# ShawnHuang497/MedPLIB

Hardware: AMD Instinct MI355X
Metric: train samples/sec (img+64tok) (higher is better)
Workload: dtype bf16

## Files before the change

### include/medplib_hip.h

```cpp
#ifndef MEDPLIB_HIP_H
#define MEDPLIB_HIP_H
#include <stddef.h>
#include <stdint.h>

#ifdef __cplusplus
extern "C" {
#endif

typedef struct ihipStream_t* hipStream_t;

#define MP_OK 0
#define MP_ERR_SHAPE (-1)
#define MP_ERR_DTYPE (-2)
#define MP_ERR_WORKSPACE (-3)
#define MP_ERR_LAUNCH (-4)
#define MP_ERR_ARG (-5)
#define MP_BF16 0
#define MP_F32 1
#define MP_ACT_NONE 0
#define MP_ACT_RELU 1
#define MP_ACT_GELU 2
#define MP_ACT_QUICK_GELU 3
#define MP_ACT_SILU 4
#define MP_ACT_SWIGLU_PAIR 5

int mp_version(void);
const char* mp_arch(void);
const char* mp_last_error_string(void);
int mp_profile_marker(int tag, hipStream_t stream);


int mp_gemm_bf16_nt(const void* A, int64_t lda, const void* W, int64_t ldw, void* C, int64_t ldc, const float* bias,
                    const void* residual, int64_t ldr, int M, int N, int K, int act, int out_dtype, float alpha,
                    const int* m_dev, hipStream_t stream);
int mp_gemm_qkv_rope_bf16(const void* A, int64_t lda, const void* Wi, int64_t ldw, void* C, int64_t ldc, const float* cos_t,
                          const float* sin_t, int M, int N, int K, int seq, int pos_offset, int head_dim, hipStream_t stream);
int mp_gemm_qkv_rope_bounded_bf16(const void* A, int64_t lda, const void* Wi, int64_t ldw, void* C, int64_t ldc, const float* cos_t,
                                  const float* sin_t, int M, int N, int K, int seq, int pos_offset, int head_dim, int table_rows,
                                  hipStream_t stream);
int mp_gemm_swiglu_keep_bf16(const void* A, int64_t lda, const void* W, int64_t ldw, void* act_out, int64_t ld_act, void* gu_out,
                             int64_t ld_gu, int M, int N, int K, hipStream_t stream);
int mp_gemm_last_kernel(void);
int mp_gemm_tile_policy(int mode);
int64_t mp_gemm_tail_wait(int64_t cycles);
int mp_gemm_bf16_nt_batched(const void* A, int64_t lda, int64_t strideA, const void* W, int64_t ldw, int64_t strideW,
                            void* C, int64_t ldc, int64_t strideC, const float* bias, int64_t strideBias, int batch,
                            int M, int N, int K, int act, int out_dtype, const int* m_dev, hipStream_t stream);

int mp_gemm_bf16_nt_batched_res(const void* A, int64_t lda, int64_t strideA, const void* W, int64_t ldw, int64_t strideW, void* C,
                                int64_t ldc, int64_t strideC, const void* residual, int64_t ldr, int64_t strideR, int batch, int M, int N,
                                int K, const int* m_dev, hipStream_t stream);

int mp_gemm_bf16_nt_batched_rows(const void* A, int64_t lda, int64_t strideA, const int* a_rows, const void* W, int64_t ldw,
                                 int64_t strideW, void* C, int64_t ldc, int64_t strideC, const int* c_rows, const float* c_scale,
                                 const void* residual, int64_t ldr, int rows_stride, int batch, int M, int N, int K, int act,
                                 const int* m_dev, hipStream_t stream);

int mp_gemv_bf16(const void* x, int64_t ldx, const void* W, int64_t ldw, int64_t strideW, void* y, int64_t ldy, const float* bias,
                 const void* residual, int64_t ldr, const int* w_index, const float* row_scale, const int* row_keep, int M, int N, int K,
                 int act, int out_dtype, float alpha, hipStream_t stream);
int mp_gemv_top2_gate_up_bf16(const void* x, int64_t ldx, const void* W, int64_t ldw, int64_t strideW, void* act, int64_t ldact,
                              const int* expert, const int* slot, int tokens, int N, int K, hipStream_t stream);
int mp_gemv_top2_down_bf16(const void* act, int64_t ldact, const void* W, int64_t ldw, int64_t strideW, void* y, int64_t ldy,
                           const void* residual, int64_t ldr, const int* expert, const int* slot, const float* weight, int tokens, int N,
                           int K, hipStream_t stream);
int mp_gemv_rmsnorm_bf16(const void* x, int64_t ldx, const float* norm_w, float eps, const void* W, int64_t ldw, void* y, int64_t ldy,
                         int M, int N, int K, int act, int out_dtype, hipStream_t stream);
int mp_gemv_rmsnorm_rope_append_bf16(const void* x, int64_t ldx, const float* norm_w, float eps, const void* W_qkv, int64_t ldw, void* qkv,
                                     int64_t ldy, const float* cos_t, const float* sin_t, void* cache_k, void* cache_v, const int* pos_dev,
                                     int M, int heads, int head_dim, int K, int64_t cache_batch_stride, int64_t cache_seq_stride,
                                     hipStream_t stream);
#define MP_POS_ERR_TABLE 1
#define MP_POS_ERR_CACHE 2
#define MP_POS_ERR_BEAM 4
int mp_gemv_rmsnorm_rope_append_bounded_bf16(const void* x, int64_t ldx, const float* norm_w, float eps, const void* W_qkv, int64_t ldw,
                                             void* qkv, int64_t ldy, const float* cos_t, const float* sin_t, void* cache_k, void* cache_v,
                                             const int* pos_dev, int M, int heads, int head_dim, int K, int64_t cache_batch_stride,
// ... 293 lines not shown
```

### medplib_amd/csrc/gemm320_bf16.hip

```cpp
#include "gemm_common.h"
#include <stdlib.h>
#include <algorithm>

namespace {

constexpr int BM3 = 320, BN3 = 256, BK3 = 64, NT3 = 512;
constexpr int A_BYTES = BM3 * 128, B_BYTES = BN3 * 128, STAGE3 = A_BYTES + B_BYTES;

__device__ __forceinline__ int lds_off3(int r, int c) { return r * 128 + ((c ^ (r & 7)) << 4); }

#define MP3_BAR()                          \
  do {                                     \
    asm volatile("" ::: "memory");         \
    __builtin_amdgcn_sched_barrier(0);     \
    __builtin_amdgcn_s_barrier();          \
    __builtin_amdgcn_sched_barrier(0);     \
    asm volatile("" ::: "memory");         \
  } while (0)
#define MP3_LGKM0() asm volatile("s_waitcnt lgkmcnt(0)" ::: "memory")

constexpr int EPI_PLAIN = 0, EPI_ROPE = 1, EPI_SWIGLU = 2, EPI_COMBINE = 3, EPI_RELU = 4, EPI_GELU = 5;
template <int EPI>
__device__ __forceinline__ void gemm320_epilogue(const GemmArgs& g, f32x4 (&acc)[5][8], int batch, int M, int N, int m0, int n0, int wr, int wc,
                                                 int fr, int fq, unsigned items = 0xfffffu) {
  bf16_t* Cb = reinterpret_cast<bf16_t*>(g.C) + batch * g.sC;
  const int cw = n0 + wc * 128;
  const int c8 = pair_col8(fq);
  if constexpr (EPI == EPI_SWIGLU) {
    float rsc[5] = {1.f, 1.f, 1.f, 1.f, 1.f};
    if (g.a_scale) {
#pragma unroll
      for (int i = 0; i < 5; ++i) {
        const int row = m0 + wr * 80 + i * 16 + fr;
        if (row < M) rsc[i] = g.a_scale[g.a_rows ? g.a_rows[batch * g.rows_stride + row] : row];
      }
    }
#pragma unroll
    for (int i = 0; i < 5; ++i) {
      const int row = m0 + wr * 80 + i * 16 + fr;
#pragma unroll
      for (int jb = 0; jb < 2; ++jb) {
        if (!((items >> (i * 4 + jb * 2)) & 1u)) continue;
        bf16x4 o[2];
#pragma unroll
        for (int jj = 0; jj < 2; ++jj)
#pragma unroll
          for (int r = 0; r < 4; ++r) {
            acc[i][jb * 4 + jj][r] *= rsc[i];
            acc[i][jb * 4 + jj + 2][r] *= rsc[i];
            const float gf = (float)(bf16_t)acc[i][jb * 4 + jj][r];
            const float uf = (float)(bf16_t)acc[i][jb * 4 + jj + 2][r];
            o[jj][r] = (bf16_t)(gf * mp_sigmoid_fast(gf) * uf);
          }
        const bf16x8 p = pair_swap16(o[0], o[1]);
        if (row < M) *reinterpret_cast<bf16x8*>(Cb + (int64_t)row * g.ldc + (cw >> 1) + jb * 32 + c8) = p;
        if (g.keep_gu) {
          const bf16x8 pg = pair_swap16(round4(acc[i][jb * 4]), round4(acc[i][jb * 4 + 1])), pu = pair_swap16(round4(acc[i][jb * 4 + 2]), round4(acc[i][jb * 4 + 3]));
          if (row < M) {
            *reinterpret_cast<bf16x8*>(g.keep_gu + (int64_t)row * g.ld_gu + cw + jb * 64 + c8) = pg;
            *reinterpret_cast<bf16x8*>(g.keep_gu + (int64_t)row * g.ld_gu + cw + jb * 64 + 32 + c8) = pu;
          }
        }
      }
      __builtin_amdgcn_sched_barrier(0);
    }
    return;
  }
  if constexpr (EPI == EPI_COMBINE) {
    bf16_t* Cs = reinterpret_cast<bf16_t*>(g.C);
    int orow[5];
    float sc[5];
#pragma unroll
    for (int i = 0; i < 5; ++i) {
      const int row = m0 + wr * 80 + i * 16 + fr;
      orow[i] = row < M ? g.c_rows[batch * g.rows_stride + row] : -1;
    }
#pragma unroll
    for (int i = 0; i < 5; ++i) sc[i] = (orow[i] >= 0 && g.c_scale) ? g.c_scale[orow[i]] : 1.f;
#pragma unroll
    for (int h = 0; h < 2; ++h) {
      bf16x8 rv[5][2];
#pragma unroll
      for (int i = 0; i < 5; ++i)
#pragma unroll
        for (int jp = 0; jp < 2; ++jp) {
          const int col = cw + (h * 2 + jp) * 32 + c8;
          rv[i][jp] = bf16x8{};
          if (g.residual && orow[i] >= 0 && ((items >> (i * 4 + h * 2 + jp)) & 1u))
            rv[i][jp] = *reinterpret_cast<const bf16x8*>(g.residual + (int64_t)orow[i] * g.ldr + col);
        }
      __builtin_amdgcn_sched_barrier(0);
#pragma unroll
      for (int i = 0; i < 5; ++i)
#pragma unroll
        for (int jp = 0; jp < 2; ++jp) {
          const int col = cw + (h * 2 + jp) * 32 + c8;
          const bf16x8 p = pair_swap16(round4(acc[i][(h * 2 + jp) * 2]), round4(acc[i][(h * 2 + jp) * 2 + 1]));
          bf16x8 o;
#pragma unroll
          for (int e = 0; e < 8; ++e) {
            float v = (float)p[e] * sc[i];
            if (g.residual) v += (float)rv[i][jp][e];
            o[e] = (bf16_t)v;
          }
          if (orow[i] >= 0 && ((items >> (i * 4 + h * 2 + jp)) & 1u)) *reinterpret_cast<bf16x8*>(Cs + (int64_t)orow[i] * g.ldc + col) = o;
        }
      __builtin_amdgcn_sched_barrier(0);
    }
    return;
  }
  if constexpr (EPI == EPI_ROPE) {
    const bool is_v = n0 >= (N / 3) * 2;
    const int head0 = (cw >> 7) << 7;
    f32x4 cs[2][2][2], sn[2][2][2];
    float rsc[2] = {1.f, 1.f};
    auto fetch = [&](int i, int buf) {
      const int row = m0 + wr * 80 + i * 16 + fr;
      const int pos = (row < M ? row : 0) % g.rope_seq + g.rope_pos0;
      if (g.a_scale) rsc[buf] = g.a_scale[row < M ? row : 0];
#pragma unroll
      for (int jb = 0; jb < 2; ++jb)
#pragma unroll
        for (int jj = 0; jj < 2; ++jj) {
          const int dim = jb * 32 + jj * 16 + fq * 4;
          cs[buf][jb][jj] = *reinterpret_cast<const f32x4*>(g.rope_cos + (int64_t)pos * 64 + dim);
          sn[buf][jb][jj] = *reinterpret_cast<const f32x4*>(g.rope_sin + (int64_t)pos * 64 + dim);
        }
    };
    fetch(0, 0);
#pragma unroll
    for (int i = 0; i < 5; ++i) {
      if (i + 1 < 5) fetch(i + 1, (i + 1) & 1);
      __builtin_amdgcn_sched_barrier(0);
      const int row = m0 + wr * 80 + i * 16 + fr;
#pragma unroll
      for (int jb = 0; jb < 2; ++jb) {
        bf16x4 olo[2], ohi[2];
#pragma unroll
        for (int jj = 0; jj < 2; ++jj) {
          const bf16x4 qa = round4(acc[i][jb * 4 + jj] * rsc[i & 1]), qb = round4(acc[i][jb * 4 + jj + 2] * rsc[i & 1]);
#pragma unroll
          for (int r = 0; r < 4; ++r) {
            const float a = (float)qa[r], b = (float)qb[r];
            const bf16_t rlo = (bf16_t)(a * cs[i & 1][jb][jj][r] - b * sn[i & 1][jb][jj][r]);
            const bf16_t rhi = (bf16_t)(b * cs[i & 1][jb][jj][r] + a * sn[i & 1][jb][jj][r]);
            olo[jj][r] = is_v ? qa[r] : rlo;
            ohi[jj][r] = is_v ? qb[r] : rhi;
          }
        }
        const bf16x8 plo = pair_swap16(olo[0], olo[1]), phi = pair_swap16(ohi[0], ohi[1]);
        const int col_lo = (is_v ? cw + jb * 64 : head0 + jb * 32) + c8;
        const int col_hi = (is_v ? cw + jb * 64 + 32 : head0 + 64 + jb * 32) + c8;
        if (row < M) {
          *reinterpret_cast<bf16x8*>(Cb + (int64_t)row * g.ldc + col_lo) = plo;
          *reinterpret_cast<bf16x8*>(Cb + (int64_t)row * g.ldc + col_hi) = phi;
        }
      }
      __builtin_amdgcn_sched_barrier(0);
    }
    return;
  }
  const float* bias0 = g.bias ? g.bias + batch * g.sBias : nullptr;
  if (g.alpha != 1.f || bias0) {
#pragma unroll
    for (int j = 0; j < 8; ++j) {
      f32x4 bv = {0.f, 0.f, 0.f, 0.f};
      if (bias0) {
#pragma unroll
        for (int r = 0; r < 4; ++r) { const int col = cw + j * 16 + fq * 4 + r; bv[r] = col < N ? bias0[col] : 0.f; }
      }
#pragma unroll
      for (int i = 0; i < 5; ++i) acc[i][j] = acc[i][j] * g.alpha + bv;
    }
  }
#define MP3_ACT_SWEEP(EXPR)                                                          \
  _Pragma("unroll") for (int i = 0; i < 5; ++i) _Pragma("unroll") for (int j = 0; j < 8; ++j) {                    \
    _Pragma("unroll") for (int r = 0; r < 4; ++r) { const float v = acc[i][j][r]; acc[i][j][r] = (EXPR); }         \
    __builtin_amdgcn_sched_barrier(0);                                                                             \
  }
  if constexpr (EPI == EPI_RELU) { MP3_ACT_SWEEP(fmaxf(v, 0.f)) }
  else if constexpr (EPI == EPI_GELU) { MP3_ACT_SWEEP(gelu_erf_fast(v)) }
  else if (g.act == ACT_QUICK_GELU) { MP3_ACT_SWEEP(v * mp_sigmoid_fast(v, 1.702f)) }
#undef MP3_ACT_SWEEP
  const bf16_t* R = g.residual ? g.residual + batch * g.sR : nullptr;
#pragma unroll
  for (int h = 0; h < 2; ++h) {
    bf16x8 rv[5][2];
    if (R) {
#pragma unroll
      for (int i = 0; i < 5; ++i) {
        const int row = m0 + wr * 80 + i * 16 + fr;
#pragma unroll
        for (int jp = 0; jp < 2; ++jp) {
          const int col = cw + (h * 2 + jp) * 32 + c8;
          rv[i][jp] = bf16x8{};
          if (row < M && col < N && ((items >> (i * 4 + h * 2 + jp)) & 1u)) rv[i][jp] = *reinterpret_cast<const bf16x8*>(R + (int64_t)row * g.ldr + col);
        }
      }
      __builtin_amdgcn_sched_barrier(0);
    }
#pragma unroll
    for (int i = 0; i < 5; ++i) {
      const int row = m0 + wr * 80 + i * 16 + fr;
#pragma unroll
      for (int jp = 0; jp < 2; ++jp) {
        const int col = cw + (h * 2 + jp) * 32 + c8;
        bf16x8 p = pair_swap16(round4(acc[i][(h * 2 + jp) * 2]), round4(acc[i][(h * 2 + jp) * 2 + 1]));
        if (R) {
#pragma unroll
          for (int e = 0; e < 8; ++e) p[e] = (bf16_t)((float)p[e] + (float)rv[i][jp][e]);
        }
        if (row < M && col < N && ((items >> (i * 4 + h * 2 + jp)) & 1u)) *reinterpret_cast<bf16x8*>(Cb + (int64_t)row * g.ldc + col) = p;
      }
    }
    __builtin_amdgcn_sched_barrier(0);
  }
}

constexpr int MAX_FLAT_BATCH3 = 8;
template <int EPI>
__global__ __launch_bounds__(NT3, 1) void gemm320_bf16_nt_kernel(GemmArgs g) {
  extern __shared__ __attribute__((aligned(16))) char smem[];
  const int N = g.N;
  const int tiles_n = N / BN3;
  int T = 0;
  int pre[MAX_FLAT_BATCH3];
#pragma unroll
  for (int b = 0; b < MAX_FLAT_BATCH3; ++b) {
    pre[b] = T;
    if (b < g.nbatch) {
      const int Mb = g.m_dev ? min(g.M, g.m_dev[b * g.m_dev_stride]) : g.M;
      T += ((Mb + BM3 - 1) / BM3) * tiles_n;
    }
  }
  const int C = g.n_cu;
  const int full = (T / C) * C, rem = T - full;
  const int nt_all = g.K / BK3;
  int S = 1;
  if (g.ws && rem > 0 && rem * 2 <= C) S = max(1, min(min(min(C / rem, g.max_split), nt_all / 4), EPI == EPI_SWIGLU ? 10 : 20));
  const int bid = blockIdx.x;
  if (bid >= full + rem * S) return;
  int flat, split = 0;
  if (bid < full) {
    flat = (bid & 7) * (full >> 3) + (bid >> 3);
  } else {
    const int r = bid - full;
    if (S == 1 && (rem & 7) == 0) {
      flat = full + (r & 7) * (rem >> 3) + (r >> 3);
    } else {
      flat = full + r % rem;
      split = r / rem;
    }
  }
  const bool is_split = (bid >= full) && S > 1;
  int batch = 0, pbase = 0;
#pragma unroll
  for (int b = 1; b < MAX_FLAT_BATCH3; ++b) if (b < g.nbatch && flat >= pre[b]) { batch = b; pbase = pre[b]; }
  const int lid = flat - pbase;
  const int M = g.m_dev ? min(g.M, g.m_dev[batch * g.m_dev_stride]) : g.M;
  const int tiles_m = (M + BM3 - 1) / BM3;
  const int GROUP_M = g.group_m;
  const int per_group = GROUP_M * tiles_n;
  const int grp = lid / per_group;
  const int first_m = grp * GROUP_M;
  const int gsz = min(tiles_m - first_m, GROUP_M);
  const int tm = first_m + (lid % per_group) % gsz, tn = (lid % per_group) / gsz;
  const int m0 = tm * BM3, n0 = tn * BN3;
  int kt0 = 0, nt = nt_all;
  if (is_split) {
    const int base = nt_all / S, extra = nt_all % S;
    kt0 = split * base + min(split, extra);
    nt = base + (split < extra ? 1 : 0);
  }
  const int k_byte0 = kt0 * (BK3 * 2);

  const int tid = threadIdx.x;
  const int lane = tid & 63;
  const int wave = __builtin_amdgcn_readfirstlane(tid >> 6);
  const int wc = wave >> 2, wr = wave & 3;
  const int fr = lane & 15, fq = lane >> 4;

  const int sub_row = lane >> 3;
  const int src_c = (lane & 7) ^ sub_row;
  const __amdgpu_buffer_rsrc_t rs_a = __builtin_amdgcn_make_buffer_rsrc(const_cast<bf16_t*>(g.A + batch * g.sA), 0,
                                          g.a_rows ? 0x7ffffff0 : (int)(((int64_t)(M - 1) * g.lda + g.K) * 2), 0x00020000);
  const __amdgpu_buffer_rsrc_t rs_w = __builtin_amdgcn_make_buffer_rsrc(const_cast<bf16_t*>(g.W + batch * g.sW), 0, (int)(((int64_t)(N - 1) * g.ldw + g.K) * 2), 0x00020000);
  const int w_lane = (int)((sub_row * g.ldw + src_c * 8) * 2);
  const int w_row_bytes = (int)(g.ldw * 2);
  int a_off[5];
#pragma unroll
  for (int i = 0; i < 5; ++i) {
    int row = m0 + (wave + 8 * i) * 8 + sub_row;
    if (g.a_rows) row = g.a_rows[batch * g.rows_stride + min(row, M - 1)];
    a_off[i] = (int)(((int64_t)row * g.lda + src_c * 8) * 2);
  }
  int b_piece[4];
#pragma unroll
  for (int k = 0; k < 4; ++k) {
    const int e = 2 * wave + (k & 1);
    b_piece[k] = (e & 7) + (e >> 3) * 16 + (k >> 1) * 8;
  }
  auto dma_a = [&](int i, int t) {
    __builtin_amdgcn_raw_ptr_buffer_load_lds(rs_a, (__attribute__((address_space(3))) void*)(smem + (t & 1) * STAGE3 + (wave + 8 * i) * 1024), 16,
                                             a_off[i], k_byte0 + t * (BK3 * 2), 0, 0);
  };
  auto dma_b = [&](int k, int t) {
    __builtin_amdgcn_raw_ptr_buffer_load_lds(rs_w, (__attribute__((address_space(3))) void*)(smem + (t & 1) * STAGE3 + A_BYTES + b_piece[k] * 1024), 16,
                                             w_lane, (n0 + b_piece[k] * 8) * w_row_bytes + k_byte0 + t * (BK3 * 2), 0, 0);
  };

  f32x4 acc[5][8];
#pragma unroll
  for (int i = 0; i < 5; ++i)
#pragma unroll
    for (int j = 0; j < 8; ++j) acc[i][j] = f32x4{0.f, 0.f, 0.f, 0.f};
  bf16x8 fa[5][2], fb[4][2];
  const int a_rd0 = (wr * 80 + fr) * 128 + ((fq ^ (fr & 7)) << 4), a_rd1 = (wr * 80 + fr) * 128 + (((4 + fq) ^ (fr & 7)) << 4);
  const int b_rd0 = A_BYTES + (wc * 128 + fr) * 128 + ((fq ^ (fr & 7)) << 4), b_rd1 = A_BYTES + (wc * 128 + fr) * 128 + (((4 + fq) ^ (fr & 7)) << 4);
  auto load_a = [&](const char* st) {
#pragma unroll
    for (int i = 0; i < 5; ++i) {
      fa[i][0] = *reinterpret_cast<const bf16x8*>(st + a_rd0 + i * 2048);
      fa[i][1] = *reinterpret_cast<const bf16x8*>(st + a_rd1 + i * 2048);
    }
  };
  auto load_b = [&](int hn, const char* st) {
#pragma unroll
    for (int j = 0; j < 4; ++j) {
      fb[j][0] = *reinterpret_cast<const bf16x8*>(st + b_rd0 + (hn * 64 + j * 16) * 128);
      fb[j][1] = *reinterpret_cast<const bf16x8*>(st + b_rd1 + (hn * 64 + j * 16) * 128);
    }
  };
#ifndef MP3_PRIO
#define MP3_PRIO 0
#endif
#define MP3_MFMA_40(HN)                                                                                     \
  do {                                                                                                      \
    if (MP3_PRIO == 0) __builtin_amdgcn_s_setprio(1);                                                       \
    _Pragma("unroll") for (int kk = 0; kk < 2; ++kk)                                                        \
      _Pragma("unroll") for (int i = 0; i < 5; ++i)                                                         \
        _Pragma("unroll") for (int j = 0; j < 4; ++j)                                                       \
          acc[i][(HN) * 4 + j] = __builtin_amdgcn_mfma_f32_16x16x32_bf16(fb[j][kk], fa[i][kk], acc[i][(HN) * 4 + j], 0, 0, 0); \
    if (MP3_PRIO == 0) __builtin_amdgcn_s_setprio(0);                                                       \
    MP3_BAR();                                                                                              \
  } while (0)

#pragma unroll
  for (int i = 0; i < 5; ++i) dma_a(i, 0);
#pragma unroll
  for (int k = 0; k < 4; ++k) dma_b(k, 0);
  if (nt > 1) {
#pragma unroll
    for (int i = 0; i < 5; ++i) dma_a(i, 1);
    dma_b(0, 1); dma_b(1, 1);
    asm volatile("s_waitcnt vmcnt(7)" ::: "memory");
  } else {
    asm volatile("s_waitcnt vmcnt(0)" ::: "memory");
  }
  MP3_BAR();
  if (wc == 1) MP3_BAR();
  if (MP3_PRIO == 2 && wc == 1) __builtin_amdgcn_s_setprio(1);

  for (int t = 0; t < nt; ++t) {
    const char* st = smem + (t & 1) * STAGE3;
    const bool n1 = (t + 1 < nt), n2 = (t + 2 < nt);
    load_b(0, st);
    load_a(st);
    __builtin_amdgcn_sched_barrier(0);
    if (n1) { dma_b(2, t + 1); dma_b(3, t + 1); }
    MP3_LGKM0();
    MP3_BAR();
    MP3_MFMA_40(0);
    load_b(1, st);
    __builtin_amdgcn_sched_barrier(0);
    if (n2) {
#pragma unroll
      for (int i = 0; i < 5; ++i) dma_a(i, t + 2);
      dma_b(0, t + 2); dma_b(1, t + 2);
      asm volatile("s_waitcnt vmcnt(7)" ::: "memory");
    } else {
      asm volatile("s_waitcnt vmcnt(0)" ::: "memory");
    }
    MP3_LGKM0();
    MP3_BAR();
    MP3_MFMA_40(1);
  }
  if (wc == 0) MP3_BAR();
  if (MP3_PRIO == 2) __builtin_amdgcn_s_setprio(0);
  unsigned items = 0xfffffu;
  if (is_split) {
    typedef __attribute__((ext_vector_type(4))) unsigned int u32x4;
    constexpr int SLAB = BM3 * BN3 * 4;
    const int tail = flat - full;
    float* tile_ws = g.ws + ((int64_t)tail * S) * (BM3 * BN3);
    const __amdgpu_buffer_rsrc_t rs = __builtin_amdgcn_make_buffer_rsrc(tile_ws, 0, S * SLAB, 0x00020000);
    const int my_off = split * SLAB + tid * 16;
#pragma unroll
    for (int i = 0; i < 5; ++i)
#pragma unroll
      for (int j = 0; j < 8; ++j)
        __builtin_amdgcn_raw_buffer_store_b128(__builtin_bit_cast(u32x4, acc[i][j]), rs, my_off + (i * 8 + j) * (NT3 * 16), 0, 16);
    asm volatile("s_waitcnt vmcnt(0)" ::: "memory");
    __syncthreads();
    int* arrive = g.tickets + tail;
    int* depart = g.tickets + 128 + tail;
    int* mode = g.tickets + 256 + tail;
    constexpr int MODE_COOP = 1, MODE_LAST = 2;
    int* s_flag = reinterpret_cast<int*>(smem);
    if (tid == 0) {
      __hip_atomic_fetch_add(arrive, 1, __ATOMIC_RELAXED, __HIP_MEMORY_SCOPE_AGENT);
      const long long t0 = __builtin_amdgcn_s_memtime();
      int m = 0, seen = 0;
      for (;;) {
        seen = __hip_atomic_load(arrive, __ATOMIC_RELAXED, __HIP_MEMORY_SCOPE_AGENT);
        if (seen >= S) break;
        m = __hip_atomic_load(mode, __ATOMIC_RELAXED, __HIP_MEMORY_SCOPE_AGENT);
        if (m) break;
        if (__builtin_amdgcn_s_memtime() - t0 > g.tail_wait) break;
        __builtin_amdgcn_s_sleep(8);
      }
      if (!m) {
        int expected = 0;
        const int want = seen >= S ? MODE_COOP : MODE_LAST;
        m = __hip_atomic_compare_exchange_strong(mode, &expected, want, __ATOMIC_RELAXED, __ATOMIC_RELAXED, __HIP_MEMORY_SCOPE_AGENT) ? want : expected;
      }
      int last = 0;
      if (m == MODE_LAST) last = __hip_atomic_fetch_add(depart, 1, __ATOMIC_RELAXED, __HIP_MEMORY_SCOPE_AGENT) == S - 1;
      s_flag[0] = m | (last << 8);
    }
    __syncthreads();
    const int decided = s_flag[0];
    __syncthreads();
    const bool coop = (decided & 0xff) == MODE_COOP;
    if (!coop && !(decided >> 8)) return;
    constexpr int N_ITEMS = (EPI == EPI_SWIGLU) ? 10 : 20;
    items = 0;
#pragma unroll
    for (int it = 0; it < N_ITEMS; ++it)
      if (!coop || it % S == split) items |= (EPI == EPI_SWIGLU) ? (3u << (2 * it)) : (1u << it);
#pragma unroll
    for (int i = 0; i < 5; ++i)
#pragma unroll
      for (int j = 0; j < 8; ++j) acc[i][j] = f32x4{0.f, 0.f, 0.f, 0.f};
    for (int sp = 0; sp < S; ++sp) {
      const int base = sp * SLAB + tid * 16;
#pragma unroll
      for (int it = 0; it < 20; ++it) {
        if (!((items >> it) & 1u)) continue;
        const int i = it >> 2, j0 = (it & 3) * 2;
        u32x4 t[2];
#pragma unroll
        for (int q = 0; q < 2; ++q) t[q] = __builtin_amdgcn_raw_buffer_load_b128(rs, base + (i * 8 + j0 + q) * (NT3 * 16), 0, 16);
#pragma unroll
        for (int q = 0; q < 2; ++q) acc[i][j0 + q] += __builtin_bit_cast(f32x4, t[q]);
      }
    }
    asm volatile("s_waitcnt vmcnt(0)" ::: "memory");
    __syncthreads();
    if (tid == 0) {
      const bool rearm = coop ? (__hip_atomic_fetch_add(depart, 1, __ATOMIC_RELAXED, __HIP_MEMORY_SCOPE_AGENT) == S - 1) : true;
      if (rearm) {
        __hip_atomic_store(depart, 0, __ATOMIC_RELAXED, __HIP_MEMORY_SCOPE_AGENT);
        __hip_atomic_store(mode, 0, __ATOMIC_RELAXED, __HIP_MEMORY_SCOPE_AGENT);
        __hip_atomic_store(arrive, 0, __ATOMIC_RELAXED, __HIP_MEMORY_SCOPE_AGENT);
      }
    }
  }
  int tid2 = threadIdx.x;
  asm volatile("" : "+v"(tid2));
  gemm320_epilogue<EPI>(g, acc, batch, M, N, m0, n0, (tid2 >> 6) & 3, tid2 >> 8, tid2 & 15, (tid2 >> 4) & 3, items);
}

}

bool mp_gemm320_eligible(const GemmArgs& g, int batch) {
  if (batch < 1 || batch > MAX_FLAT_BATCH3 || g.out_f32) return false;
  if (g.keep_gu && (batch != 1 || (g.ld_gu & 7) || (reinterpret_cast<uintptr_t>(g.keep_gu) & 15))) return false;
  if (!(g.act == ACT_NONE || g.act == ACT_QUICK_GELU || g.act == ACT_ROPE_QK || g.act == ACT_SWIGLU_PAIR || g.act == ACT_RELU || g.act == ACT_GELU)) return false;
  if ((g.act == ACT_RELU || g.act == ACT_GELU) && (g.c_rows || g.a_rows)) return false;
  if (g.act == ACT_ROPE_QK && (batch != 1 || g.m_dev || g.a_rows || g.c_rows)) return false;
  if (g.act == ACT_SWIGLU_PAIR && (g.c_rows || g.residual || g.bias || g.alpha != 1.f || ((g.N >> 1) & 7))) return false;
  if (g.c_rows && (g.act != ACT_NONE || g.bias || g.alpha != 1.f)) return false;
  if (g.a_scale && !(g.act == ACT_ROPE_QK || g.act == ACT_SWIGLU_PAIR)) return false;
  if (g.N % BN3 || g.K % BK3 || g.M < (mp_gemm_policy_whole_tiles() ? BM3 : 1024)) return false;
  if ((g.ldc & 7) || (reinterpret_cast<uintptr_t>(g.C) & 15) || (g.sC & 7)) return false;
  if (g.residual && ((g.ldr & 7) || (reinterpret_cast<uintptr_t>(g.residual) & 15) || (g.sR & 7))) return false;
  const int64_t a_rows_bound = g.a_rows ? (int64_t)batch * g.M * 4 : (int64_t)g.M + 320;
  if (a_rows_bound * g.lda * 2 >= (1ll << 31) || (int64_t)g.N * g.ldw * 2 >= (1ll << 31)) return false;
  return true;
}

int mp_gemm320_subwave_split(const GemmArgs& g, int batch) {
  static int on = -1;
  if (on < 0) { const char* e = getenv("MP_GEMM320_SUBWAVE"); on = (e && atoi(e) == 0) ? 0 : 1; }
  if (!on || batch != 1 || g.m_dev || g.act == ACT_ROPE_QK || g.M < 1024 || g.K < 8192) return 1;
  if (mp_gemm_policy_whole_tiles()) return 1;
  const int C = std::min(mp_device_cus(), 256);
  const int64_t tiles = (int64_t)mp_cdiv(g.M, BM3) * (g.N / BN3);
  if (tiles * 2 > C || tiles * 4 <= C) return 1;
  const int64_t S = std::min<int64_t>(C / tiles, g.K / BK3 / 4);
  if (S < 2 || S * tiles * 10 < (int64_t)C * 9) return 1;
  return (int)S;
}

int mp_launch_gemm320(const GemmArgs& g0, int batch, hipStream_t stream) {
  static bool attr = false;
  if (!attr) {
    (void)hipFuncSetAttribute((const void*)gemm320_bf16_nt_kernel<EPI_PLAIN>, hipFuncAttributeMaxDynamicSharedMemorySize, 2 * STAGE3);
    (void)hipFuncSetAttribute((const void*)gemm320_bf16_nt_kernel<EPI_ROPE>, hipFuncAttributeMaxDynamicSharedMemorySize, 2 * STAGE3);
    (void)hipFuncSetAttribute((const void*)gemm320_bf16_nt_kernel<EPI_SWIGLU>, hipFuncAttributeMaxDynamicSharedMemorySize, 2 * STAGE3);
    (void)hipFuncSetAttribute((const void*)gemm320_bf16_nt_kernel<EPI_COMBINE>, hipFuncAttributeMaxDynamicSharedMemorySize, 2 * STAGE3);
    (void)hipFuncSetAttribute((const void*)gemm320_bf16_nt_kernel<EPI_RELU>, hipFuncAttributeMaxDynamicSharedMemorySize, 2 * STAGE3);
    (void)hipFuncSetAttribute((const void*)gemm320_bf16_nt_kernel<EPI_GELU>, hipFuncAttributeMaxDynamicSharedMemorySize, 2 * STAGE3);
    attr = true;
  }
  GemmArgs g = g0;
  g.nbatch = batch;
  g.n_cu = std::min(mp_device_cus(), 256);
  static int max_split = -1;
  if (max_split < 0) { const char* e = getenv("MP_GEMM320_MAX_SPLIT"); max_split = (e && atoi(e) >= 1) ? atoi(e) : 10; }
  static int dense_split = -1;
  if (dense_split < 0) { const char* e = getenv("MP_GEMM320_DENSE_SPLIT"); dense_split = (e && atoi(e) == 0) ? 0 : 1; }
  const int64_t dense_tiles = (int64_t)mp_cdiv(g.M, BM3) * (g.N / BN3);
  g.max_split = (batch > 1 || g.m_dev) ? max_split : ((dense_split && (dense_tiles > g.n_cu || mp_gemm320_subwave_split(g, batch) > 1)) ? max_split : 1);
  if (g.act == ACT_ROPE_QK) g.max_split = 1;
  if (mp_gemm_stream_registered(stream) || mp_gemm_policy_whole_tiles()) g.max_split = 1;
  g.tail_wait = mp_gemm_tail_wait_value();
  int64_t ws_bytes = 0;
  mp_gemm_split_workspace(stream, &g.ws, &g.tickets, &ws_bytes);
  if (!g.ws || ws_bytes < (int64_t)g.n_cu * BM3 * BN3 * 4) { g.ws = nullptr; g.tickets = nullptr; g.max_split = 1; }
  const int64_t host_tiles = (int64_t)mp_cdiv(g.M, BM3) * (g.N / BN3) * batch;
  const int64_t host_rem = host_tiles % g.n_cu;
  const bool may_split = g.max_split > 1 && (g.m_dev || (host_rem > 0 && host_rem * 2 <= g.n_cu));
  const dim3 grid((unsigned)(host_tiles + (may_split ? g.n_cu : 0)));
#define MP3_GO(E) hipLaunchKernelGGL(gemm320_bf16_nt_kernel<E>, grid, dim3(NT3), 2 * STAGE3, stream, g)
  if (g.act == ACT_ROPE_QK) MP3_GO(EPI_ROPE);
  else if (g.act == ACT_SWIGLU_PAIR) MP3_GO(EPI_SWIGLU);
  else if (g.c_rows) MP3_GO(EPI_COMBINE);
  else if (g.act == ACT_RELU) MP3_GO(EPI_RELU);
  else if (g.act == ACT_GELU) MP3_GO(EPI_GELU);
  else MP3_GO(EPI_PLAIN);
#undef MP3_GO
  return mp_check_launch("mp_gemm_bf16_nt(320)");
}
```

### medplib_amd/csrc/gemm_common.h

```cpp
#pragma once
#include "common.h"

enum { ACT_NONE = 0, ACT_RELU = 1, ACT_GELU = 2, ACT_QUICK_GELU = 3, ACT_SILU = 4,
       ACT_SWIGLU_PAIR = 5,
       ACT_ROPE_QK = 6 };

struct GemmArgs {
  const bf16_t* A;  int64_t lda;
  const bf16_t* W;  int64_t ldw;
  void* C;          int64_t ldc;
  const float* bias;
  const bf16_t* residual;
  int64_t ldr;
  const int* m_dev;
  int M, N, K;
  int act;
  int out_f32;
  float alpha;
  int64_t sA, sW, sC, sR, sBias;
  int m_dev_stride;
  int group_m;
  float* ws; int* tickets;
  int n_cu;
  int nbatch;
  int max_split;
  long long tail_wait;
  const int* a_rows; const int* c_rows; const float* c_scale;
  int rows_stride;
  const float* rope_cos; const float* rope_sin;
  int rope_seq, rope_pos0;
  int ep8;
  bf16_t* keep_gu; int64_t ld_gu;
  const float* a_scale;
};

static __device__ __forceinline__ float gelu_erf_fast(float x) {
  const float xp = fmaxf(x, 0.f);
  const float a = fabsf(x);
  float q = fmaf(-0.0004733088717330247f, a, 0.007084553129971027f);
  q = fmaf(q, a, -0.05182736739516258f);
  q = fmaf(q, a, -0.4599924683570862f);
  q = fmaf(q, a, -1.1507878303527832f);
  q = fmaf(q, a, -1.000037670135498f);
  return fmaf(-a, __builtin_amdgcn_exp2f(q), xp);
}

static __device__ __forceinline__ float apply_act(float v, int act) {
  switch (act) {
    case ACT_RELU: return fmaxf(v, 0.f);
    case ACT_GELU: return gelu_erf_fast(v);
    case ACT_QUICK_GELU: return v * mp_sigmoid_fast(v, 1.702f);
    case ACT_SILU: return v * mp_sigmoid_fast(v);
    default: return v;
  }
}


void mp_launch_gemm128(const GemmArgs& g, int batch, bool may_split, hipStream_t stream);
int mp_launch_gemm256(const GemmArgs& g, int batch, hipStream_t stream);
// ... 21 lines not shown
```

### medplib_amd/ops.py

```python
import torch

from ._lib import lib

BF16, F32 = 0, 1
ACT_NONE, ACT_RELU, ACT_GELU, ACT_QUICK_GELU, ACT_SILU, ACT_SWIGLU_PAIR = 0, 1, 2, 3, 4, 5
SACT_NONE, SACT_RELU, SACT_GELU, SACT_SIGMOID = 0, 1, 2, 3


def _stream():
    return torch.cuda.current_stream().cuda_stream


def _p(t):
    return None if t is None else t.data_ptr()


def _chk(t, dtype, name):
    if not t.is_cuda:
        raise ValueError(f"{name}: expected a GPU tensor (medplib_amd has no CPU path)")
    if t.dtype != dtype:
        raise TypeError(f"{name}: expected {dtype}, got {t.dtype}")


def _dt(dtype):
# ... 161 lines not shown
    import functools

    @functools.wraps(fn)
    def wrapped(*args, **kwargs):
        with throughput_tiles():
            return fn(*args, **kwargs)
    return wrapped


class throughput_tiles:
    _on = None

    def __enter__(self):
        if throughput_tiles._on is None:
            import os
            throughput_tiles._on = os.environ.get("MP_TOWER_THROUGHPUT_TILES", "1") != "0"
        global _TOWER_DEPTH
        _TOWER_DEPTH += 1
        self._prev = _TILE_POLICY
        if throughput_tiles._on and self._prev == -1:
            gemm_tile_policy(3)
        return self

    def __exit__(self, *exc):
        global _TOWER_DEPTH
        _TOWER_DEPTH -= 1
        if _TILE_POLICY != self._prev:
            gemm_tile_policy(self._prev)
        return False


def gemm_tail_wait(cycles=-1):
    return int(lib().raw("mp_gemm_tail_wait")(int(cycles)))


def gemm_last_kernel():
    return int(lib().raw("mp_gemm_last_kernel")())


def gemv_rmsnorm(x, norm_w, eps, w, out_dtype=torch.bfloat16, act=ACT_NONE):
    _chk(x, torch.bfloat16, "gemv_rmsnorm.x"); _chk(w, torch.bfloat16, "gemv_rmsnorm.w"); _chk(norm_w, torch.float32, "gemv_rmsnorm.norm_w")
    M, K = x.shape
    N = w.shape[0]
    assert x.stride(1) == 1 and w.stride(1) == 1 and w.shape[1] == K and norm_w.is_contiguous() and norm_w.numel() == K
    out = torch.empty((M, N // 2 if act == ACT_SWIGLU_PAIR else N), dtype=out_dtype, device=x.device)
    lib().call("mp_gemv_rmsnorm_bf16", _p(x), x.stride(0), _p(norm_w), float(eps), _p(w), w.stride(0), _p(out), out.stride(0), M, N, K,
               int(act), _dt(out_dtype), _stream())
    return out


def gemv_rmsnorm_rope_append(x, norm_w, eps, w_qkv, cos_t, sin_t, cache_k, cache_v, pos_dev, heads, head_dim, err=None):
    _chk(x, torch.bfloat16, "gemv_rmsnorm_rope.x"); _chk(w_qkv, torch.bfloat16, "gemv_rmsnorm_rope.w"); _chk(pos_dev, torch.int32, "gemv_rmsnorm_rope.pos")
    M, K = x.shape
    assert w_qkv.shape == (3 * heads * head_dim, K) and x.stride(1) == 1 and w_qkv.stride(1) == 1
    assert cache_k.stride(3) == 1 and cache_k.stride(2) == head_dim and cache_v.stride() == cache_k.stride()
    qkv = torch.empty((M, 3 * heads * head_dim), dtype=torch.bfloat16, device=x.device)
    table_rows, cache_rows, err = _decode_bounds(cos_t, sin_t, cache_k, cache_v, err)
    lib().call("mp_gemv_rmsnorm_rope_append_bounded_bf16", _p(x), x.stride(0), _p(norm_w), float(eps), _p(w_qkv), w_qkv.stride(0), _p(qkv),
               qkv.stride(0), _p(cos_t), _p(sin_t), _p(cache_k), _p(cache_v), _p(pos_dev), M, heads, head_dim, K, cache_k.stride(0),
               cache_k.stride(1), table_rows, cache_rows, _p(err), _stream())
    return qkv


def gemv_rmsnorm_ok(M, K, head_dim=None, swiglu_n=None):
    if not (M <= 2 and K % 512 == 0 and (K // 512) in (1, 2, 4, 8, 16) and 4 * M * K * 2 <= 160 * 1024):
        return False
# ... 1388 lines not shown
```

Baseline: 138.5.

## Specialize 320-row GEMM tiles for short M edges to skip padded rows

The 320x256 GEMM kernel is templated on the number of fragment rows per wave, and tiles whose remaining M rows fit in 64/128/192/256 dispatch a short variant. That variant uses an interleaved row mapping and issues only the needed A loads and MFMAs. This is meant to remove the DMA and MFMA work on padded rows in the last M tile, which matters for ragged per-expert or short-sequence batches. In exchange it adds four more template instantiations, which cost code size and compile time. Short tiles are disabled on the wave just ahead of split tails, and an environment toggle can turn the feature off.

```diff
diff --git a/include/medplib_hip.h b/include/medplib_hip.h
--- a/include/medplib_hip.h
+++ b/include/medplib_hip.h
@@ -43,6 +43,7 @@
 int mp_gemm_last_kernel(void);
 int mp_gemm_tile_policy(int mode);
 int64_t mp_gemm_tail_wait(int64_t cycles);
+int mp_gemm320_short_tiles(int on);
 int mp_gemm_bf16_nt_batched(const void* A, int64_t lda, int64_t strideA, const void* W, int64_t ldw, int64_t strideW,
                             void* C, int64_t ldc, int64_t strideC, const float* bias, int64_t strideBias, int batch,
                             int M, int N, int K, int act, int out_dtype, const int* m_dev, hipStream_t stream);
diff --git a/medplib_amd/csrc/gemm320_bf16.hip b/medplib_amd/csrc/gemm320_bf16.hip
--- a/medplib_amd/csrc/gemm320_bf16.hip
+++ b/medplib_amd/csrc/gemm320_bf16.hip
@@ -19,25 +19,30 @@
   } while (0)
 #define MP3_LGKM0() asm volatile("s_waitcnt lgkmcnt(0)" ::: "memory")
 
+template <bool SHORT>
+__device__ __forceinline__ int tile_row3(int wr, int i, int fr) { return SHORT ? (4 * i + wr) * 16 + fr : wr * 80 + i * 16 + fr; }
+
 constexpr int EPI_PLAIN = 0, EPI_ROPE = 1, EPI_SWIGLU = 2, EPI_COMBINE = 3, EPI_RELU = 4, EPI_GELU = 5;
-template <int EPI>
-__device__ __forceinline__ void gemm320_epilogue(const GemmArgs& g, f32x4 (&acc)[5][8], int batch, int M, int N, int m0, int n0, int wr, int wc,
+template <int EPI, int R, bool SHORT>
+__device__ __forceinline__ void gemm320_epilogue(const GemmArgs& g, f32x4 (&acc)[R][8], int batch, int M, int N, int m0, int n0, int wr, int wc,
                                                  int fr, int fq, unsigned items = 0xfffffu) {
   bf16_t* Cb = reinterpret_cast<bf16_t*>(g.C) + batch * g.sC;
   const int cw = n0 + wc * 128;
   const int c8 = pair_col8(fq);
   if constexpr (EPI == EPI_SWIGLU) {
-    float rsc[5] = {1.f, 1.f, 1.f, 1.f, 1.f};
+    float rsc[R];
+#pragma unroll
+    for (int i = 0; i < R; ++i) rsc[i] = 1.f;
     if (g.a_scale) {
 #pragma unroll
-      for (int i = 0; i < 5; ++i) {
-        const int row = m0 + wr * 80 + i * 16 + fr;
+      for (int i = 0; i < R; ++i) {
+        const int row = m0 + tile_row3<SHORT>(wr, i, fr);
         if (row < M) rsc[i] = g.a_scale[g.a_rows ? g.a_rows[batch * g.rows_stride + row] : row];
       }
     }
 #pragma unroll
-    for (int i = 0; i < 5; ++i) {
-      const int row = m0 + wr * 80 + i * 16 + fr;
+    for (int i = 0; i < R; ++i) {
+      const int row = m0 + tile_row3<SHORT>(wr, i, fr);
 #pragma unroll
       for (int jb = 0; jb < 2; ++jb) {
         if (!((items >> (i * 4 + jb * 2)) & 1u)) continue;
@@ -68,20 +73,20 @@
   }
   if constexpr (EPI == EPI_COMBINE) {
     bf16_t* Cs = reinterpret_cast<bf16_t*>(g.C);
-    int orow[5];
-    float sc[5];
-#pragma unroll
-    for (int i = 0; i < 5; ++i) {
-      const int row = m0 + wr * 80 + i * 16 + fr;
+    int orow[R];
+    float sc[R];
+#pragma unroll
+    for (int i = 0; i < R; ++i) {
+      const int row = m0 + tile_row3<SHORT>(wr, i, fr);
       orow[i] = row < M ? g.c_rows[batch * g.rows_stride + row] : -1;
     }
 #pragma unroll
-    for (int i = 0; i < 5; ++i) sc[i] = (orow[i] >= 0 && g.c_scale) ? g.c_scale[orow[i]] : 1.f;
+    for (int i = 0; i < R; ++i) sc[i] = (orow[i] >= 0 && g.c_scale) ? g.c_scale[orow[i]] : 1.f;
 #pragma unroll
     for (int h = 0; h < 2; ++h) {
-      bf16x8 rv[5][2];
-#pragma unroll
-      for (int i = 0; i < 5; ++i)
+      bf16x8 rv[R][2];
+#pragma unroll
+      for (int i = 0; i < R; ++i)
 #pragma unroll
         for (int jp = 0; jp < 2; ++jp) {
           const int col = cw + (h * 2 + jp) * 32 + c8;
@@ -91,7 +96,7 @@
         }
       __builtin_amdgcn_sched_barrier(0);
 #pragma unroll
-      for (int i = 0; i < 5; ++i)
+      for (int i = 0; i < R; ++i)
 #pragma unroll
         for (int jp = 0; jp < 2; ++jp) {
           const int col = cw + (h * 2 + jp) * 32 + c8;
@@ -115,7 +120,7 @@
     f32x4 cs[2][2][2], sn[2][2][2];
     float rsc[2] = {1.f, 1.f};
     auto fetch = [&](int i, int buf) {
-      const int row = m0 + wr * 80 + i * 16 + fr;
+      const int row = m0 + tile_row3<SHORT>(wr, i, fr);
       const int pos = (row < M ? row : 0) % g.rope_seq + g.rope_pos0;
       if (g.a_scale) rsc[buf] = g.a_scale[row < M ? row : 0];
 #pragma unroll
@@ -129,10 +134,10 @@
     };
     fetch(0, 0);
 #pragma unroll
-    for (int i = 0; i < 5; ++i) {
-      if (i + 1 < 5) fetch(i + 1, (i + 1) & 1);
+    for (int i = 0; i < R; ++i) {
+      if (i + 1 < R) fetch(i + 1, (i + 1) & 1);
       __builtin_amdgcn_sched_barrier(0);
-      const int row = m0 + wr * 80 + i * 16 + fr;
+      const int row = m0 + tile_row3<SHORT>(wr, i, fr);
 #pragma unroll
       for (int jb = 0; jb < 2; ++jb) {
         bf16x4 olo[2], ohi[2];
@@ -170,11 +175,11 @@
         for (int r = 0; r < 4; ++r) { const int col = cw + j * 16 + fq * 4 + r; bv[r] = col < N ? bias0[col] : 0.f; }
       }
 #pragma unroll
-      for (int i = 0; i < 5; ++i) acc[i][j] = acc[i][j] * g.alpha + bv;
+      for (int i = 0; i < R; ++i) acc[i][j] = acc[i][j] * g.alpha + bv;
     }
   }
 #define MP3_ACT_SWEEP(EXPR)                                                          \
-  _Pragma("unroll") for (int i = 0; i < 5; ++i) _Pragma("unroll") for (int j = 0; j < 8; ++j) {                    \
+  _Pragma("unroll") for (int i = 0; i < R; ++i) _Pragma("unroll") for (int j = 0; j < 8; ++j) {                    \
     _Pragma("unroll") for (int r = 0; r < 4; ++r) { const float v = acc[i][j][r]; acc[i][j][r] = (EXPR); }         \
     __builtin_amdgcn_sched_barrier(0);                                                                             \
   }
@@ -182,31 +187,31 @@
   else if constexpr (EPI == EPI_GELU) { MP3_ACT_SWEEP(gelu_erf_fast(v)) }
   else if (g.act == ACT_QUICK_GELU) { MP3_ACT_SWEEP(v * mp_sigmoid_fast(v, 1.702f)) }
 #undef MP3_ACT_SWEEP
-  const bf16_t* R = g.residual ? g.residual + batch * g.sR : nullptr;
+  const bf16_t* Rs = g.residual ? g.residual + batch * g.sR : nullptr;
 #pragma unroll
   for (int h = 0; h < 2; ++h) {
-    bf16x8 rv[5][2];
-    if (R) {
-#pragma unroll
-      for (int i = 0; i < 5; ++i) {
-        const int row = m0 + wr * 80 + i * 16 + fr;
+    bf16x8 rv[R][2];
+    if (Rs) {
+#pragma unroll
+      for (int i = 0; i < R; ++i) {
+        const int row = m0 + tile_row3<SHORT>(wr, i, fr);
 #pragma unroll
         for (int jp = 0; jp < 2; ++jp) {
           const int col = cw + (h * 2 + jp) * 32 + c8;
           rv[i][jp] = bf16x8{};
-          if (row < M && col < N && ((items >> (i * 4 + h * 2 + jp)) & 1u)) rv[i][jp] = *reinterpret_cast<const bf16x8*>(R + (int64_t)row * g.ldr + col);
+          if (row < M && col < N && ((items >> (i * 4 + h * 2 + jp)) & 1u)) rv[i][jp] = *reinterpret_cast<const bf16x8*>(Rs + (int64_t)row * g.ldr + col);
         }
       }
       __builtin_amdgcn_sched_barrier(0);
     }
 #pragma unroll
-    for (int i = 0; i < 5; ++i) {
-      const int row = m0 + wr * 80 + i * 16 + fr;
+    for (int i = 0; i < R; ++i) {
+      const int row = m0 + tile_row3<SHORT>(wr, i, fr);
 #pragma unroll
       for (int jp = 0; jp < 2; ++jp) {
         const int col = cw + (h * 2 + jp) * 32 + c8;
         bf16x8 p = pair_swap16(round4(acc[i][(h * 2 + jp) * 2]), round4(acc[i][(h * 2 + jp) * 2 + 1]));
-        if (R) {
+        if (Rs) {
 #pragma unroll
           for (int e = 0; e < 8; ++e) p[e] = (bf16_t)((float)p[e] + (float)rv[i][jp][e]);
         }
@@ -218,62 +223,10 @@
 }
 
 constexpr int MAX_FLAT_BATCH3 = 8;
-template <int EPI>
-__global__ __launch_bounds__(NT3, 1) void gemm320_bf16_nt_kernel(GemmArgs g) {
-  extern __shared__ __attribute__((aligned(16))) char smem[];
-  const int N = g.N;
-  const int tiles_n = N / BN3;
-  int T = 0;
-  int pre[MAX_FLAT_BATCH3];
-#pragma unroll
-  for (int b = 0; b < MAX_FLAT_BATCH3; ++b) {
-    pre[b] = T;
-    if (b < g.nbatch) {
-      const int Mb = g.m_dev ? min(g.M, g.m_dev[b * g.m_dev_stride]) : g.M;
-      T += ((Mb + BM3 - 1) / BM3) * tiles_n;
-    }
-  }
-  const int C = g.n_cu;
-  const int full = (T / C) * C, rem = T - full;
-  const int nt_all = g.K / BK3;
-  int S = 1;
-  if (g.ws && rem > 0 && rem * 2 <= C) S = max(1, min(min(min(C / rem, g.max_split), nt_all / 4), EPI == EPI_SWIGLU ? 10 : 20));
-  const int bid = blockIdx.x;
-  if (bid >= full + rem * S) return;
-  int flat, split = 0;
-  if (bid < full) {
-    flat = (bid & 7) * (full >> 3) + (bid >> 3);
-  } else {
-    const int r = bid - full;
-    if (S == 1 && (rem & 7) == 0) {
-      flat = full + (r & 7) * (rem >> 3) + (r >> 3);
-    } else {
-      flat = full + r % rem;
-      split = r / rem;
-    }
-  }
-  const bool is_split = (bid >= full) && S > 1;
-  int batch = 0, pbase = 0;
-#pragma unroll
-  for (int b = 1; b < MAX_FLAT_BATCH3; ++b) if (b < g.nbatch && flat >= pre[b]) { batch = b; pbase = pre[b]; }
-  const int lid = flat - pbase;
-  const int M = g.m_dev ? min(g.M, g.m_dev[batch * g.m_dev_stride]) : g.M;
-  const int tiles_m = (M + BM3 - 1) / BM3;
-  const int GROUP_M = g.group_m;
-  const int per_group = GROUP_M * tiles_n;
-  const int grp = lid / per_group;
-  const int first_m = grp * GROUP_M;
-  const int gsz = min(tiles_m - first_m, GROUP_M);
-  const int tm = first_m + (lid % per_group) % gsz, tn = (lid % per_group) / gsz;
-  const int m0 = tm * BM3, n0 = tn * BN3;
-  int kt0 = 0, nt = nt_all;
-  if (is_split) {
-    const int base = nt_all / S, extra = nt_all % S;
-    kt0 = split * base + min(split, extra);
-    nt = base + (split < extra ? 1 : 0);
-  }
-  const int k_byte0 = kt0 * (BK3 * 2);
-
+template <int EPI, int R, bool SHORT>
+__device__ __forceinline__ void gemm320_tile(const GemmArgs& g, char* smem, int batch, int M, int N, int m0, int n0, int k_byte0, int nt, bool is_split,
+                                             int split, int S, int tail) {
+  static_assert(SHORT ? (R >= 1 && R < 5) : R == 5, "full tiles run five fragment rows per wave, short ones one to four");
   const int tid = threadIdx.x;
   const int lane = tid & 63;
   const int wave = __builtin_amdgcn_readfirstlane(tid >> 6);
@@ -287,9 +240,9 @@
   const __amdgpu_buffer_rsrc_t rs_w = __builtin_amdgcn_make_buffer_rsrc(const_cast<bf16_t*>(g.W + batch * g.sW), 0, (int)(((int64_t)(N - 1) * g.ldw + g.K) * 2), 0x00020000);
   const int w_lane = (int)((sub_row * g.ldw + src_c * 8) * 2);
   const int w_row_bytes = (int)(g.ldw * 2);
-  int a_off[5];
-#pragma unroll
-  for (int i = 0; i < 5; ++i) {
+  int a_off[R];
+#pragma unroll
+  for (int i = 0; i < R; ++i) {
     int row = m0 + (wave + 8 * i) * 8 + sub_row;
     if (g.a_rows) row = g.a_rows[batch * g.rows_stride + min(row, M - 1)];
     a_off[i] = (int)(((int64_t)row * g.lda + src_c * 8) * 2);
@@ -309,19 +262,20 @@
                                              w_lane, (n0 + b_piece[k] * 8) * w_row_bytes + k_byte0 + t * (BK3 * 2), 0, 0);
   };
 
-  f32x4 acc[5][8];
-#pragma unroll
-  for (int i = 0; i < 5; ++i)
+  f32x4 acc[R][8];
+#pragma unroll
+  for (int i = 0; i < R; ++i)
 #pragma unroll
     for (int j = 0; j < 8; ++j) acc[i][j] = f32x4{0.f, 0.f, 0.f, 0.f};
-  bf16x8 fa[5][2], fb[4][2];
-  const int a_rd0 = (wr * 80 + fr) * 128 + ((fq ^ (fr & 7)) << 4), a_rd1 = (wr * 80 + fr) * 128 + (((4 + fq) ^ (fr & 7)) << 4);
+  bf16x8 fa[R][2], fb[4][2];
+  constexpr int A_ROW0 = SHORT ? 16 : 80, A_STEP = SHORT ? 64 * 128 : 16 * 128;
+  const int a_rd0 = (wr * A_ROW0 + fr) * 128 + ((fq ^ (fr & 7)) << 4), a_rd1 = (wr * A_ROW0 + fr) * 128 + (((4 + fq) ^ (fr & 7)) << 4);
   const int b_rd0 = A_BYTES + (wc * 128 + fr) * 128 + ((fq ^ (fr & 7)) << 4), b_rd1 = A_BYTES + (wc * 128 + fr) * 128 + (((4 + fq) ^ (fr & 7)) << 4);
   auto load_a = [&](const char* st) {
 #pragma unroll
-    for (int i = 0; i < 5; ++i) {
-      fa[i][0] = *reinterpret_cast<const bf16x8*>(st + a_rd0 + i * 2048);
-      fa[i][1] = *reinterpret_cast<const bf16x8*>(st + a_rd1 + i * 2048);
+    for (int i = 0; i < R; ++i) {
+      fa[i][0] = *reinterpret_cast<const bf16x8*>(st + a_rd0 + i * A_STEP);
+      fa[i][1] = *reinterpret_cast<const bf16x8*>(st + a_rd1 + i * A_STEP);
     }
   };
   auto load_b = [&](int hn, const char* st) {
@@ -334,11 +288,11 @@
 #ifndef MP3_PRIO
 #define MP3_PRIO 0
 #endif
-#define MP3_MFMA_40(HN)                                                                                     \
+#define MP3_MFMA_SEG(HN)                                                                                     \
   do {                                                                                                      \
     if (MP3_PRIO == 0) __builtin_amdgcn_s_setprio(1);                                                       \
     _Pragma("unroll") for (int kk = 0; kk < 2; ++kk)                                                        \
-      _Pragma("unroll") for (int i = 0; i < 5; ++i)                                                         \
+      _Pragma("unroll") for (int i = 0; i < R; ++i)                                                         \
         _Pragma("unroll") for (int j = 0; j < 4; ++j)                                                       \
           acc[i][(HN) * 4 + j] = __builtin_amdgcn_mfma_f32_16x16x32_bf16(fb[j][kk], fa[i][kk], acc[i][(HN) * 4 + j], 0, 0, 0); \
     if (MP3_PRIO == 0) __builtin_amdgcn_s_setprio(0);                                                       \
@@ -346,14 +300,14 @@
   } while (0)
 
 #pragma unroll
-  for (int i = 0; i < 5; ++i) dma_a(i, 0);
+  for (int i = 0; i < R; ++i) dma_a(i, 0);
 #pragma unroll
   for (int k = 0; k < 4; ++k) dma_b(k, 0);
   if (nt > 1) {
 #pragma unroll
-    for (int i = 0; i < 5; ++i) dma_a(i, 1);
+    for (int i = 0; i < R; ++i) dma_a(i, 1);
     dma_b(0, 1); dma_b(1, 1);
-    asm volatile("s_waitcnt vmcnt(7)" ::: "memory");
+    asm volatile("s_waitcnt vmcnt(%0)" ::"n"(R + 2) : "memory");
   } else {
     asm volatile("s_waitcnt vmcnt(0)" ::: "memory");
   }
@@ -370,20 +324,20 @@
     if (n1) { dma_b(2, t + 1); dma_b(3, t + 1); }
     MP3_LGKM0();
     MP3_BAR();
-    MP3_MFMA_40(0);
+    MP3_MFMA_SEG(0);
     load_b(1, st);
     __builtin_amdgcn_sched_barrier(0);
     if (n2) {
 #pragma unroll
-      for (int i = 0; i < 5; ++i) dma_a(i, t + 2);
+      for (int i = 0; i < R; ++i) dma_a(i, t + 2);
       dma_b(0, t + 2); dma_b(1, t + 2);
-      asm volatile("s_waitcnt vmcnt(7)" ::: "memory");
+      asm volatile("s_waitcnt vmcnt(%0)" ::"n"(R + 2) : "memory");
     } else {
       asm volatile("s_waitcnt vmcnt(0)" ::: "memory");
     }
     MP3_LGKM0();
     MP3_BAR();
-    MP3_MFMA_40(1);
+    MP3_MFMA_SEG(1);
   }
   if (wc == 0) MP3_BAR();
   if (MP3_PRIO == 2) __builtin_amdgcn_s_setprio(0);
@@ -391,12 +345,11 @@
   if (is_split) {
     typedef __attribute__((ext_vector_type(4))) unsigned int u32x4;
     constexpr int SLAB = BM3 * BN3 * 4;
-    const int tail = flat - full;
     float* tile_ws = g.ws + ((int64_t)tail * S) * (BM3 * BN3);
     const __amdgpu_buffer_rsrc_t rs = __builtin_amdgcn_make_buffer_rsrc(tile_ws, 0, S * SLAB, 0x00020000);
     const int my_off = split * SLAB + tid * 16;
 #pragma unroll
-    for (int i = 0; i < 5; ++i)
+    for (int i = 0; i < R; ++i)
 #pragma unroll
       for (int j = 0; j < 8; ++j)
         __builtin_amdgcn_raw_buffer_store_b128(__builtin_bit_cast(u32x4, acc[i][j]), rs, my_off + (i * 8 + j) * (NT3 * 16), 0, 16);
@@ -439,13 +392,13 @@
     for (int it = 0; it < N_ITEMS; ++it)
       if (!coop || it % S == split) items |= (EPI == EPI_SWIGLU) ? (3u << (2 * it)) : (1u << it);
 #pragma unroll
-    for (int i = 0; i < 5; ++i)
+    for (int i = 0; i < R; ++i)
 #pragma unroll
       for (int j = 0; j < 8; ++j) acc[i][j] = f32x4{0.f, 0.f, 0.f, 0.f};
     for (int sp = 0; sp < S; ++sp) {
       const int base = sp * SLAB + tid * 16;
 #pragma unroll
-      for (int it = 0; it < 20; ++it) {
+      for (int it = 0; it < R * 4; ++it) {
         if (!((items >> it) & 1u)) continue;
         const int i = it >> 2, j0 = (it & 3) * 2;
         u32x4 t[2];
@@ -468,7 +421,78 @@
   }
   int tid2 = threadIdx.x;
   asm volatile("" : "+v"(tid2));
-  gemm320_epilogue<EPI>(g, acc, batch, M, N, m0, n0, (tid2 >> 6) & 3, tid2 >> 8, tid2 & 15, (tid2 >> 4) & 3, items);
+  gemm320_epilogue<EPI, R, SHORT>(g, acc, batch, M, N, m0, n0, (tid2 >> 6) & 3, tid2 >> 8, tid2 & 15, (tid2 >> 4) & 3, items);
+}
+
+template <int EPI>
+__global__ __launch_bounds__(NT3, 1) void gemm320_bf16_nt_kernel(GemmArgs g) {
+  extern __shared__ __attribute__((aligned(16))) char smem[];
+  const int N = g.N;
+  const int tiles_n = N / BN3;
+  int T = 0;
+  int pre[MAX_FLAT_BATCH3];
+#pragma unroll
+  for (int b = 0; b < MAX_FLAT_BATCH3; ++b) {
+    pre[b] = T;
+    if (b < g.nbatch) {
+      const int Mb = g.m_dev ? min(g.M, g.m_dev[b * g.m_dev_stride]) : g.M;
+      T += ((Mb + BM3 - 1) / BM3) * tiles_n;
+    }
+  }
+  const int C = g.n_cu;
+  const int full = (T / C) * C, rem = T - full;
+  const int nt_all = g.K / BK3;
+  int S = 1;
+  if (g.ws && rem > 0 && rem * 2 <= C) S = max(1, min(min(min(C / rem, g.max_split), nt_all / 4), EPI == EPI_SWIGLU ? 10 : 20));
+  const int bid = blockIdx.x;
+  if (bid >= full + rem * S) return;
+  int flat, split = 0;
+  if (bid < full) {
+    flat = (bid & 7) * (full >> 3) + (bid >> 3);
+  } else {
+    const int r = bid - full;
+    if (S == 1 && (rem & 7) == 0) {
+      flat = full + (r & 7) * (rem >> 3) + (r >> 3);
+    } else {
+      flat = full + r % rem;
+      split = r / rem;
+    }
+  }
+  const bool is_split = (bid >= full) && S > 1;
+  int batch = 0, pbase = 0;
+#pragma unroll
+  for (int b = 1; b < MAX_FLAT_BATCH3; ++b) if (b < g.nbatch && flat >= pre[b]) { batch = b; pbase = pre[b]; }
+  const int lid = flat - pbase;
+  const int M = g.m_dev ? min(g.M, g.m_dev[batch * g.m_dev_stride]) : g.M;
+  const int tiles_m = (M + BM3 - 1) / BM3;
+  const int GROUP_M = g.group_m;
+  const int per_group = GROUP_M * tiles_n;
+  const int grp = lid / per_group;
+  const int first_m = grp * GROUP_M;
+  const int gsz = min(tiles_m - first_m, GROUP_M);
+  const int tm = first_m + (lid % per_group) % gsz, tn = (lid % per_group) / gsz;
+  const int m0 = tm * BM3, n0 = tn * BN3;
+  int kt0 = 0, nt = nt_all;
+  if (is_split) {
+    const int base = nt_all / S, extra = nt_all % S;
+    kt0 = split * base + min(split, extra);
+    nt = base + (split < extra ? 1 : 0);
+  }
+  const int k_byte0 = kt0 * (BK3 * 2);
+
+  const bool ahead_of_split_tail = S > 1 && bid >= full - C && bid < full;
+  const int R = (g.short_tiles && !ahead_of_split_tail) ? (min(BM3, M - m0) + 63) >> 6 : 5;
+  const int tail = flat - full;
+#define MP3_TILE(RR, SH) gemm320_tile<EPI, RR, SH>(g, smem, batch, M, N, m0, n0, k_byte0, nt, is_split, split, S, tail)
+  if (__builtin_expect(R == 5, 1)) { MP3_TILE(5, false); return; }
+  switch (R) {
+    case 1: MP3_TILE(1, true); break;
+    case 2: MP3_TILE(2, true); break;
+    case 3: MP3_TILE(3, true); break;
+    case 4: MP3_TILE(4, true); break;
+    default: break;
+  }
+#undef MP3_TILE
 }
 
 }
@@ -503,6 +527,17 @@
   return (int)S;
 }
 
+static int g_short_tiles = -1;
+static int short_tiles_value() {
+  if (g_short_tiles < 0) { const char* e = getenv("MP_GEMM320_SHORT"); g_short_tiles = (e && atoi(e) == 0) ? 0 : 1; }
+  return g_short_tiles;
+}
+extern "C" int mp_gemm320_short_tiles(int on) {
+  const int prev = short_tiles_value();
+  if (on >= 0) g_short_tiles = on ? 1 : 0;
+  return prev;
+}
+
 int mp_launch_gemm320(const GemmArgs& g0, int batch, hipStream_t stream) {
   static bool attr = false;
   if (!attr) {
@@ -526,6 +561,7 @@
   if (g.act == ACT_ROPE_QK) g.max_split = 1;
   if (mp_gemm_stream_registered(stream) || mp_gemm_policy_whole_tiles()) g.max_split = 1;
   g.tail_wait = mp_gemm_tail_wait_value();
+  g.short_tiles = short_tiles_value();
   int64_t ws_bytes = 0;
   mp_gemm_split_workspace(stream, &g.ws, &g.tickets, &ws_bytes);
   if (!g.ws || ws_bytes < (int64_t)g.n_cu * BM3 * BN3 * 4) { g.ws = nullptr; g.tickets = nullptr; g.max_split = 1; }
diff --git a/medplib_amd/csrc/gemm_common.h b/medplib_amd/csrc/gemm_common.h
--- a/medplib_amd/csrc/gemm_common.h
+++ b/medplib_amd/csrc/gemm_common.h
@@ -25,6 +25,7 @@
   int nbatch;
   int max_split;
   long long tail_wait;
+  int short_tiles;
   const int* a_rows; const int* c_rows; const float* c_scale;
   int rows_stride;
   const float* rope_cos; const float* rope_sin;
diff --git a/medplib_amd/ops.py b/medplib_amd/ops.py
--- a/medplib_amd/ops.py
+++ b/medplib_amd/ops.py
@@ -217,6 +217,10 @@
 
 def gemm_tail_wait(cycles=-1):
     return int(lib().raw("mp_gemm_tail_wait")(int(cycles)))
+
+
+def gemm320_short_tiles(on=-1):
+    return int(lib().raw("mp_gemm320_short_tiles")(int(on)))
 
 
 def gemm_last_kernel():
```

Measured after the change: 139.5 (median of 6 runs). No clear change (+0.7%).
